# Christopher-Wang/DistriFlow

Hardware: AMD Instinct MI355X
Metric: images/sec (whole node), MNIST CNN sync-SGD at 1/2/4/8 MI355X; async speedup (higher is better)
Workload: dtype bf16; 1 GPU; model=lenet5, global_batch=4096, per_gpu_batch=4096, parallelism=dp1, optimizer=sgd, graph=full, steps_per_graph=64, p2p_reason=single rank, step=train+reduce/update, params=61706

## Files before the change

### csrc/lenet_fused.hip

```cpp
#include "common.h"
#include "diag.h"
#include "kernels.h"
#include "lenet_frag.h"
#include "ll_exchange.h"
#include "optim_device.h"
#include "ps_device.h"

#include <algorithm>
#include <cstdlib>
#include <vector>

namespace dfa {
namespace {

constexpr int IMG = 8;
constexpr int NT = 512;
constexpr int NW = NT / 64;
constexpr int ccdiv(int a, int b) { return (a + b - 1) / b; }
constexpr int XS_ELEMS = IMG * 1024 + 32;
constexpr int OFF_XS = 0;
constexpr int OFF_P1 = OFF_XS + XS_ELEMS * 2;
constexpr int OFF_C1 = OFF_P1 + IMG * 196 * 16;
constexpr int DC2_RS = 104;
constexpr int NM = IMG * DC2_RS;
constexpr int OFF_K = OFF_C1 + IMG * 196 * 4;
constexpr int OFF_PX = OFF_K + 32;
constexpr int OFF_FT = OFF_PX + NM * 2;
constexpr int OFF_W = OFF_FT + 98 * 2 * 16;
constexpr int OFF_KZ = OFF_W + 128;
constexpr int OFF_U = OFF_KZ + 32;
constexpr int OFF_XS1 = OFF_U + 32;
constexpr int LD0 = 424, LD1 = 136, LD2 = 104, LD3 = 40;
constexpr int OFF_H0 = OFF_U;
constexpr int OFF_H1 = OFF_H0 + IMG * LD0 * 2;
constexpr int OFF_H2 = OFF_H1 + IMG * LD1 * 2;
constexpr int OFF_Z3 = OFF_H2 + IMG * LD2 * 2;
constexpr int OFF_Z2 = OFF_Z3 + IMG * LD3 * 2;
constexpr int OFF_Z1 = OFF_Z2 + IMG * LD2 * 2;
constexpr int OFF_ZR = OFF_Z1 + IMG * LD1 * 2;
constexpr int OFF_LG = OFF_ZR + LD0 * 2;
constexpr int OFF_C2 = OFF_LG + IMG * 16 * 4;
constexpr int U_DENSE = OFF_C2 + IMG * 25 * 16 - OFF_U;
constexpr int OFF_DC2 = OFF_U;
constexpr int U_DC2 = NM * 16 * 2;
constexpr int OFF_RED = OFF_XS1 + XS_ELEMS * 2;
constexpr int U_G = 32 + XS_ELEMS * 2 + 4 * 16 * 32 * 4;
__device__ __forceinline__ int dc2_swz(int t) { return t ^ ((t >> 3) & 7); }
constexpr int cmax(int a, int b) { return a > b ? a : b; }
constexpr int NFP1 = (FR_C2 - FR_C1) * 64, NFP2 = (FR_DG - FR_C2) * 64;
constexpr int OFF_FC1 = OFF_XS1;
constexpr int OFF_FC2 = OFF_U + U_DENSE;
constexpr int U_FC2 = U_DENSE + NFP2 * 16;
static_assert(FR_C1 == 0 && FR_C2 - FR_C1 == 15 && FR_DG - FR_C2 == 7, "phase 0 stages fragments 0 .. 21 as one range");
static_assert(OFF_FC1 + NFP1 * 16 <= OFF_XS1 + (XS_ELEMS / 8 - 1) * 16, "build_shift1 overwrites the conv1 fragments");
constexpr int OFF_DB = OFF_U + (cmax(cmax(cmax(U_DENSE, U_DC2), U_G), U_FC2) + 15) / 16 * 16;
constexpr int OFF_ST = OFF_DB + 864;
constexpr int LDS_BYTES = OFF_ST + 128;
static_assert(OFF_U == OFF_C1 + IMG * 196 * 4 + 128 + 98 * 2 * 16 + 800 * 2 + 128 && OFF_U % 16 == 0 && OFF_KZ % 16 == 0 && OFF_H1 % 16 == 0 && OFF_ZR % 16 == 0 && OFF_C2 % 16 == 0 && OFF_RED % 16 == 0 && OFF_DB % 16 == 0 && OFF_ST % 16 == 0 &&
                  OFF_PX % 16 == 0 && OFF_W % 16 == 0 && OFF_FC1 % 16 == 0 && OFF_FC2 % 16 == 0,
              "LDS carve must stay 16-byte aligned");
static_assert(2 * LDS_BYTES <= 160 * 1024, "two workgroups per CU");

typedef __bf16 bf16x4_vs __attribute__((__vector_size__(8)));

#define LN_STAMP(slot)                                                            \
  do {                                                                            \
    if (stamps) {                                                                 \
      __builtin_amdgcn_sched_barrier(0);                                          \
      unsigned long long t_;                                                      \
      asm volatile("s_memtime %0\n\ts_waitcnt lgkmcnt(0)" : "=s"(t_)::"memory"); \
      __builtin_amdgcn_sched_barrier(0);                                          \
      if (threadIdx.x == 0) STMP[(slot)] = t_;                                    \
    }                                                                             \
  } while (0)

template <int CTRL>
__device__ __forceinline__ float dpp_f(float v) {
  return __builtin_bit_cast(float, __builtin_amdgcn_update_dpp(0, __builtin_bit_cast(int, v), CTRL, 0xf, 0xf, false));
}
__device__ __forceinline__ float row16_max(float v) {
  v = fmaxf(v, dpp_f<0xB1>(v));
  v = fmaxf(v, dpp_f<0x4E>(v));
  v = fmaxf(v, dpp_f<0x141>(v));
  return fmaxf(v, dpp_f<0x140>(v));
}
__device__ __forceinline__ float row16_sum(float v) {
  v += dpp_f<0xB1>(v);
  v += dpp_f<0x4E>(v);
  v += dpp_f<0x141>(v);
  return v + dpp_f<0x140>(v);
}

__device__ __forceinline__ bf16x4 tr_read(const bf16* p) {
  auto* lp = (__attribute__((address_space(3))) bf16*)(const_cast<bf16*>(p));
  const bf16x4_vs v =
      __builtin_amdgcn_ds_read_tr16_b64_v4bf16(reinterpret_cast<__attribute__((address_space(3))) bf16x4_vs*>(lp));
  return __builtin_bit_cast(bf16x4, v);
}
__device__ __forceinline__ bf16x8 cat8(bf16x4 a, bf16x4 b) {
  bf16x8 r;
#pragma unroll
  for (int e = 0; e < 4; ++e) {
    r[e] = a[e];
    r[e + 4] = b[e];
  }
  return r;
}
__device__ __forceinline__ bf16x8 ld8(const bf16* p) { return *reinterpret_cast<const bf16x8*>(p); }
__device__ __forceinline__ void st8(bf16* p, const bf16x8& v) { *reinterpret_cast<bf16x8*>(p) = v; }
__device__ __forceinline__ bf16x8 zero8() {
  bf16x8 z;
#pragma unroll
  for (int e = 0; e < 8; ++e) z[e] = (bf16)0.f;
  return z;
}

__device__ __forceinline__ void build_shift1(const bf16* Xs, bf16* Xs1) {
  for (int t = threadIdx.x; t < XS_ELEMS / 8 - 1; t += NT) {
    const uint4 lo = *reinterpret_cast<const uint4*>(Xs + 8 * t);
    const unsigned nx = *reinterpret_cast<const unsigned*>(Xs + 8 * t + 8);
    uint4 o;
    o.x = __builtin_amdgcn_alignbyte(lo.y, lo.x, 2);
    o.y = __builtin_amdgcn_alignbyte(lo.z, lo.y, 2);
    o.z = __builtin_amdgcn_alignbyte(lo.w, lo.z, 2);
    o.w = __builtin_amdgcn_alignbyte(nx, lo.w, 2);
    *reinterpret_cast<uint4*>(Xs1 + 8 * t) = o;
  }
}

__device__ __forceinline__ void pool4(float a00, float a01, float a10, float a11, float& best, unsigned& code) {
  best = a00;
  code = 0;
  if (a01 > best) { best = a01; code = 1; }
  if (a10 > best) { best = a10; code = 2; }
  if (a11 > best) { best = a11; code = 3; }
  if (!(best > 0.f)) { best = 0.f; code = 4; }
}

template <int KS, int NTW>
struct DenseFrags {
  bf16x8 b[NTW][KS];
};
template <int KS, int NTW>
__device__ __forceinline__ void dense_load(DenseFrags<KS, NTW>& f, const bf16x8* __restrict__ W, int ntiles) {
  const int lane = threadIdx.x & 63, w = threadIdx.x >> 6;
#pragma unroll
  for (int tt = 0; tt < NTW; ++tt) {
    const int t = w + NW * tt;
    if (t < ntiles) {
#pragma unroll
      for (int s = 0; s < KS; ++s) f.b[tt][s] = W[(t * KS + s) * 64 + lane];
    }
  }
}

__device__ __forceinline__ void act_store4(bf16* __restrict__ T, int ldt, int n, int c0, int nlive, const float (&v)[4]) {
  if (nlive >= 4) {
    bf16x4 pk;
#pragma unroll
    for (int r = 0; r < 4; ++r) pk[r] = f2bf(v[r]);
    *reinterpret_cast<bf16x4*>(T + lenet_act_pos(n, c0, ldt)) = pk;
  } else {
    for (int r = 0; r < 4; ++r)
      if (r < nlive) T[lenet_act_pos(n, c0 + r, ldt)] = f2bf(v[r]);
  }
}

template <int KS, int NTW>
__device__ __forceinline__ void dense_fwd(const DenseFrags<KS, NTW>& f, const bf16* A, int lda, const bf16* zr,
                                          const float* __restrict__ bias, int N, bool relu, bf16* out, int ldo,
                                          float* out32, bf16* __restrict__ hT, int ldt, int r0, int rows) {
  const int lane = threadIdx.x & 63, w = threadIdx.x >> 6, i = lane & 15, g = lane >> 4;
  const int ntiles = (N + 15) / 16;
  const bf16* arow = (i < IMG ? A + i * lda : zr) + 8 * g;
#pragma unroll
  for (int tt = 0; tt < NTW; ++tt) {
    const int t = w + NW * tt;
    if (t >= ntiles) break;
    const int n = 16 * t + i;
    f32x4 acc = {0.f, 0.f, 0.f, 0.f};
#pragma unroll
    for (int s = 0; s < KS; ++s) acc = mfma16x16x32(ld8(arow + 32 * s), f.b[tt][s], acc);
    if (g >= 2) continue;
    const float bv = (bias != nullptr && n < N) ? bias[n] : 0.f;
    float v[4];
#pragma unroll
    for (int r = 0; r < 4; ++r) {
      v[r] = acc[r] + bv;
      if (relu) v[r] = fmaxf(v[r], 0.f);
      if (n >= N) v[r] = 0.f;
      const int row = 4 * g + r;
      if (out) out[row * ldo + n] = f2bf(v[r]);
      if (out32) out32[row * 16 + (n & 15)] = v[r];
    }
    if (hT != nullptr && n < N) act_store4(hT, ldt, n, r0 + 4 * g, rows - 4 * g, v);
  }
}

template <int KS, int NTW>
__device__ __forceinline__ void dense_bwd(const DenseFrags<KS, NTW>& f, const bf16* dZ, int ldz, const bf16* zr,
                                          int K, const bf16* mask, int ldm, bf16* out, int ldo,
                                          bf16* __restrict__ gT, int ldt, int r0, int rows) {
  const int lane = threadIdx.x & 63, w = threadIdx.x >> 6, i = lane & 15, g = lane >> 4;
  const int ktiles = (K + 15) / 16;
  const bf16* zrow = (i < IMG ? dZ + i * ldz : zr) + 8 * g;
#pragma unroll
  for (int tt = 0; tt < NTW; ++tt) {
    const int t = w + NW * tt;
    if (t >= ktiles) break;
    const int j = 16 * t + i;
    f32x4 acc = {0.f, 0.f, 0.f, 0.f};
#pragma unroll
    for (int s = 0; s < KS; ++s) acc = mfma16x16x32(ld8(zrow + 32 * s), f.b[tt][s], acc);
    if (g >= 2) continue;
    float v[4];
#pragma unroll
    for (int r = 0; r < 4; ++r) {
      const int row = 4 * g + r;
      v[r] = acc[r];
      if (mask != nullptr && !((float)mask[row * ldm + j] > 0.f)) v[r] = 0.f;
      if (j >= K) v[r] = 0.f;
      out[row * ldo + j] = f2bf(v[r]);
    }
    if (gT != nullptr && j < K) act_store4(gT, ldt, j, r0 + 4 * g, rows - 4 * g, v);
  }
}

__device__ __forceinline__ int lenet_img_group(int b, int nb) {
  const int per = nb / 8;
  if (b >= 8 * per) return b;
  return (b & 7) * per + (b >> 3);
}

__device__ __forceinline__ void lenet_ps_owner_decide(const PSArgs& p, unsigned* s_cnt) {
  const int k = threadIdx.x;
  if (k < p.nshards) {
    const unsigned ep = __hip_atomic_load(p.scratch + kPSEpoch, __ATOMIC_RELAXED, __HIP_MEMORY_SCOPE_AGENT) + 1u;
    const unsigned R = (unsigned)p.owner_ring;
    const unsigned pre = __hip_atomic_load(p.pref + k, __ATOMIC_RELAXED, __HIP_MEMORY_SCOPE_SYSTEM);
    unsigned P = 0, n = 0, c = pre, free_ = 0;
    if (__hip_atomic_compare_exchange_strong(p.dlock + k, &free_, (unsigned)p.rank + 1u, __ATOMIC_RELAXED,
                                             __ATOMIC_RELAXED, __HIP_MEMORY_SCOPE_SYSTEM)) {
      P = __hip_atomic_load(p.pref + k, __ATOMIC_RELAXED, __HIP_MEMORY_SCOPE_SYSTEM);
      const unsigned* fl = ps_inbox_flags(p, k);
      while (n < R && n < 255u &&
             __hip_atomic_load(const_cast<unsigned*>(fl) + (P + n) % R, __ATOMIC_RELAXED, __HIP_MEMORY_SCOPE_SYSTEM) ==
                 P + n + 1u)
        ++n;
      if (n == 0) __hip_atomic_store(p.dlock + k, 0u, __ATOMIC_RELAXED, __HIP_MEMORY_SCOPE_SYSTEM);
      c = P + n;
    }
    __hip_atomic_store(ps_owner_drain_words(p) + k, ps_owner_word(ep, n, P), __ATOMIC_RELAXED, __HIP_MEMORY_SCOPE_AGENT);
    s_cnt[k] = c;
  }
  __syncthreads();
  if (threadIdx.x == 0) {
    unsigned cnt = 0xffffffffu;
    for (int j = 0; j < p.nshards; ++j) cnt = s_cnt[j] < cnt ? s_cnt[j] : cnt;
    const unsigned dec = __hip_atomic_load(p.scratch + kPSDecision, __ATOMIC_RELAXED, __HIP_MEMORY_SCOPE_AGENT) & 7u;
    if (dec == kPSAccept && cnt == p.scratch[kPSSeq]) cnt += 1u;
    if (dec == kPSAccept || dec == kPSReject) ps_note_refresh(p, cnt);
  }
}

__device__ __forceinline__ void lenet_ps_admission(const PSArgs& p, bool excl) {
  const long long bid = *p.bid_out;
  const unsigned applied0 = ps_read_applied(p);
  const unsigned ep = __hip_atomic_load(p.scratch + kPSEpoch, __ATOMIC_RELAXED, __HIP_MEMORY_SCOPE_AGENT) + 1u;
  const unsigned dec = ps_admit(p, false);
  const bool owner = p.owner_ring > 0;
  if (!owner && (dec == kPSAccept || dec == kPSReject)) ps_note_refresh(p, applied0 + (dec == kPSAccept ? 1u : 0u));
  __hip_atomic_store(p.scratch + kPSDecision, (ep << 3) | dec, __ATOMIC_RELAXED, __HIP_MEMORY_SCOPE_AGENT);
  if (excl) {
    __hip_atomic_store(p.scratch + kPSEpoch, ep, __ATOMIC_RELAXED, __HIP_MEMORY_SCOPE_AGENT);
    if (dec == kPSAccept) ps_publish_applied(p);
  }
  if (dec == kPSAccept && p.done_epoch != nullptr) complete_microbatch(p, bid);
}

template <bool TRIM>
__global__ void __launch_bounds__(NT, 2 * NT / 256) lenet_train_kernel(LeNetArgs a) {
  if ((int)blockIdx.x >= a.nblk) {
    if (a.ps_admit && threadIdx.x == 0) lenet_ps_admission(a.ps, a.ps_excl != 0);
    return;
  }
  extern __shared__ __attribute__((aligned(16))) char smem[];
  bf16* Xs = reinterpret_cast<bf16*>(smem + OFF_XS);
  bf16* Xs1 = reinterpret_cast<bf16*>(smem + OFF_XS1);
  bf16* P1 = reinterpret_cast<bf16*>(smem + OFF_P1);
  unsigned* C1 = reinterpret_cast<unsigned*>(smem + OFF_C1);
  bf16* KO = reinterpret_cast<bf16*>(smem + OFF_K);
  unsigned char* FT = reinterpret_cast<unsigned char*>(smem + OFF_FT);
  unsigned short* PX = reinterpret_cast<unsigned short*>(smem + OFF_PX);
  float* WS = reinterpret_cast<float*>(smem + OFF_W);
  bf16* H0 = reinterpret_cast<bf16*>(smem + OFF_H0);
  bf16* H1 = reinterpret_cast<bf16*>(smem + OFF_H1);
  bf16* H2 = reinterpret_cast<bf16*>(smem + OFF_H2);
  bf16* Z3 = reinterpret_cast<bf16*>(smem + OFF_Z3);
  bf16* Z2 = reinterpret_cast<bf16*>(smem + OFF_Z2);
  bf16* Z1 = reinterpret_cast<bf16*>(smem + OFF_Z1);
  bf16* ZR = reinterpret_cast<bf16*>(smem + OFF_ZR);
  float* LG = reinterpret_cast<float*>(smem + OFF_LG);
  unsigned char* C2 = reinterpret_cast<unsigned char*>(smem + OFF_C2);
  bf16* DC2 = reinterpret_cast<bf16*>(smem + OFF_DC2);
  float* RED = reinterpret_cast<float*>(smem + OFF_RED);

  const int tid = threadIdx.x, lane = tid & 63, w = __builtin_amdgcn_readfirstlane(tid >> 6), i = lane & 15,
            g = lane >> 4;
  const int r0 = lenet_img_group(blockIdx.x, a.nblk) * (TRIM ? a.ipw : IMG);
  const int rows = min(TRIM ? a.ipw : IMG, a.B - r0);
  const int nA = TRIM ? 2 * ((7 * rows + 1) / 2) : 56;
  const int nB = TRIM ? (13 * rows + 1) / 2 : NM / 16;
  const int nE = TRIM ? ((13 * rows + 3) / 4 + 1) / 2 * 2 : NM / 32;
  const int nF = TRIM ? (49 * rows + 7) / 8 : 49;
  const int nG = TRIM ? 14 * rows : IMG * 14;
  const bf16x8* __restrict__ frag = reinterpret_cast<const bf16x8*>(a.frag);
  float* part = a.conv_part + (long long)blockIdx.x * kLeNetConvStride;
  unsigned long long* const stamps = a.stamps;
  unsigned long long* const STMP = reinterpret_cast<unsigned long long*>(smem + OFF_ST);
  LN_STAMP(0);

  const int ximg = tid / 28, xrow = tid - 28 * (tid / 28);
  const bool xload = tid < IMG * 28 && ximg < rows;
  const bool lload = tid >= 256 && tid < 256 + IMG && tid - 256 < rows;
  long long xsrc = 0, lsrc = 0;
  if (xload) xsrc = a.idx ? a.idx[r0 + ximg] : (long long)(r0 + ximg);
  if (lload) lsrc = a.idx ? a.idx[r0 + tid - 256] : (long long)(r0 + tid - 256);
  uint4 tabv = {0u, 0u, 0u, 0u};
  if (tid < 98 * 2) tabv = reinterpret_cast<const uint4*>(a.ftab)[tid];
  else if (tid >= 264 && tid < 264 + NM / 8) tabv = reinterpret_cast<const uint4*>(a.pxtab)[tid - 264];
  static_assert(98 * 2 <= 256 && 264 + NM / 8 <= 448 && 448 + 22 <= NT, "phase 0 staging thread ranges");
  float biasv = 0.f, dbv = 0.f;
  if (tid >= 448 && tid < 448 + 22) biasv = *(tid < 454 ? a.b1 + (tid - 448) : a.b2 + (tid - 454));
  if (tid < 214) dbv = *(tid < 120 ? a.d1b + tid : (tid < 204 ? a.d2b + (tid - 120) : a.d3b + (tid - 204)));
  constexpr int NFK = ccdiv(NFP1 + NFP2, NT);
  bf16x8 fv[NFK];
#pragma unroll
  for (int k = 0; k < NFK; ++k) fv[k] = frag[FR_C1 * 64 + min(tid + NT * k, NFP1 + NFP2 - 1)];
  const int lbl = a.labels[lsrc < 0 ? 0 : (lsrc >= a.nrows ? a.nrows - 1 : lsrc)];
  unsigned xv[14];
  {
    const long long src = xsrc < 0 ? 0 : (xsrc >= a.nrows ? a.nrows - 1 : xsrc);
    const int xr = xload ? xrow : 0;
    if (a.x_u8 != nullptr) {
      const unsigned* p = reinterpret_cast<const unsigned*>(a.x_u8 + src * 784 + xr * 28);
#pragma unroll
      for (int k = 0; k < 7; ++k) xv[k] = p[k];
    } else {
      const uint2* p = reinterpret_cast<const uint2*>(a.x_bf + src * 784 + xr * 28);
#pragma unroll
      for (int k = 0; k < 7; ++k) {
        const uint2 v = p[k];
        xv[2 * k] = v.x;
        xv[2 * k + 1] = v.y;
      }
    }
  }
  const bf16x8 z8 = zero8();
  bf16x8 one6 = z8;
  one6[6] = (bf16)1.f;
  for (int e = tid; e < (OFF_K - OFF_XS) / 16; e += NT)
    st8(Xs + 8 * e, (e >= OFF_P1 / 16 && e < OFF_C1 / 16) ? one6 : z8);
  static_assert(OFF_FC2 + NFP2 * 16 == OFF_DB, "the conv2 fragment image ends the union");
  if (tid < (OFF_FC1 - OFF_U) / 16) st8(reinterpret_cast<bf16*>(smem + OFF_U) + 8 * tid, z8);
  for (int e = (OFF_FC1 - OFF_U) / 16 + NFP1 + tid; e < (OFF_FC2 - OFF_U) / 16; e += NT)
    st8(reinterpret_cast<bf16*>(smem + OFF_U) + 8 * e, z8);
#pragma unroll
  for (int k = 0; k < NFK; ++k) {
    const int p = tid + NT * k;
    if (p < NFP1) st8(reinterpret_cast<bf16*>(smem + OFF_FC1) + 8 * p, fv[k]);
    else if (p < NFP1 + NFP2) st8(reinterpret_cast<bf16*>(smem + OFF_FC2) + 8 * (p - NFP1), fv[k]);
  }
  if (tid < 2) {
    bf16x8 o;
#pragma unroll
    for (int e = 0; e < 8; ++e) o[e] = (bf16)1.f;
    st8(KO + 8 * tid, o);
  } else if (tid < 4) {
    st8(reinterpret_cast<bf16*>(smem + OFF_KZ) + 8 * (tid - 2), z8);
  }
  if (tid < 98 * 2) reinterpret_cast<uint4*>(FT)[tid] = tabv;
  else if (tid >= 264 && tid < 264 + NM / 8) reinterpret_cast<uint4*>(PX)[tid - 264] = tabv;
  if (tid >= 448 && tid < 448 + 22) WS[tid - 448] = biasv;
  float* DB = reinterpret_cast<float*>(smem + OFF_DB);
  if (tid < 214) DB[tid] = dbv;
  int* LBL = reinterpret_cast<int*>(WS + 24);
  if (tid >= 256 && tid < 256 + IMG) LBL[tid - 256] = lbl;
  __syncthreads();
  bf16x8 bc[15];
#pragma unroll
  for (int f = 0; f < 15; ++f) bc[f] = ld8(reinterpret_cast<const bf16*>(smem + OFF_FC1) + 8 * (f * 64 + lane));
  if (xload) {
    unsigned* dst = reinterpret_cast<unsigned*>(Xs + ximg * 1024 + (xrow + 2) * 32 + 2);
    if (a.x_u8 != nullptr) {
#pragma unroll
      for (int k = 0; k < 7; ++k)
#pragma unroll
        for (int h = 0; h < 2; ++h) {
          const float f0 = (float)((xv[k] >> (16 * h)) & 255u) * a.scale;
          const float f1 = (float)((xv[k] >> (16 * h + 8)) & 255u) * a.scale;
          const unsigned lo = __builtin_bit_cast(unsigned short, f2bf(f0));
          const unsigned hi = __builtin_bit_cast(unsigned short, f2bf(f1));
          dst[2 * k + h] = lo | (hi << 16);
        }
    } else {
#pragma unroll
      for (int k = 0; k < 14; ++k) dst[k] = xv[k];
    }
  }
  __syncthreads();
  build_shift1(Xs, Xs1);
  __syncthreads();
  LN_STAMP(1);

  {
    const float b1c[3] = {WS[(i >> 3)], WS[2 + (i >> 3)], WS[4 + (i >> 3)]};
#pragma unroll 2
    for (int u = w; u < nA; u += NT / 64) {
      const int mt = u >> 1, x0 = (u & 1) * 16;
      const int m = 16 * mt + i;
      const int img = m / 56, rem = m - 56 * (m / 56);
      const bf16* abase = ((rem & 1) ? Xs1 : Xs) + img * 1024 + (rem >> 1) * 32 + x0 + 8 * g;
      f32x4 acc[3];
#pragma unroll
      for (int T = 0; T < 3; ++T) acc[T] = {0.f, 0.f, 0.f, 0.f};
#pragma unroll
      for (int ky = 0; ky < 5; ++ky) {
        const bf16x8 av = ld8(abase + ky * 32);
#pragma unroll
        for (int T = 0; T < 3; ++T) acc[T] = mfma16x16x32(av, bc[ky * 3 + T], acc[T]);
      }
      const int m0 = 16 * mt + 4 * g;
      const int imgo = m0 / 56, py = (m0 - 56 * (m0 / 56)) >> 2;
      const int px = (x0 >> 1) + (i & 7);
      unsigned cw = 0;
#pragma unroll
      for (int T = 0; T < 3; ++T) {
        float best;
        unsigned code;
        pool4(acc[T][0] + b1c[T], acc[T][1] + b1c[T], acc[T][2] + b1c[T], acc[T][3] + b1c[T], best, code);
        const int c = 2 * T + (i >> 3);
        if (px < 14) P1[((imgo * 14 + py) * 14 + px) * 8 + c] = f2bf(best);
        cw |= code << (3 * c);
      }
      cw |= __shfl_xor(cw, 8, 64);
      if (i < 8 && px < 14) C1[(imgo * 14 + py) * 14 + px] = cw;
    }
  }
  __syncthreads();
  LN_STAMP(2);

  bf16x8 bw[7];
#pragma unroll
  for (int s = 0; s < 7; ++s) bw[s] = ld8(reinterpret_cast<const bf16*>(smem + OFF_FC2) + 8 * (s * 64 + lane));
  DenseFrags<13, ccdiv(8, NW)> f1;
  dense_load(f1, frag + FR_D1W * 64, 8);
  {
    int toff[7];
#pragma unroll
    for (int s = 0; s < 7; ++s) {
      const int tap = 4 * s + g;
      toff[s] = tap < 25 ? ((tap / 5) * 14 + (tap - 5 * (tap / 5))) * 8 : 0;
    }
    const float b2 = WS[6 + i];
#pragma unroll 2
    for (int mt = w; mt < nB; mt += NT / 64) {
      const bf16* abase = P1 + (int)PX[16 * mt + i] * 8;
      f32x4 acc = {0.f, 0.f, 0.f, 0.f};
#pragma unroll
      for (int s = 0; s < 7; ++s) acc = mfma16x16x32(ld8(abase + toff[s]), bw[s], acc);
      const int m0 = 16 * mt + 4 * g;
      const int img0 = m0 / DC2_RS, win0 = (m0 - DC2_RS * img0) >> 2;
      float best;
      unsigned code;
      pool4(acc[0] + b2, acc[1] + b2, acc[2] + b2, acc[3] + b2, best, code);
      if (win0 < 25) {
        H0[img0 * LD0 + win0 * 16 + i] = f2bf(best);
        C2[(img0 * 25 + win0) * 16 + i] = (unsigned char)code;
      }
    }
  }
  __syncthreads();
  LN_STAMP(3);

  for (int k = tid; k < 400; k += NT) {
    if (rows == IMG) {
      bf16x8 v;
#pragma unroll
      for (int r = 0; r < IMG; ++r) v[r] = H0[r * LD0 + k];
      st8(a.h0T + lenet_act_pos(k, r0, a.ldt), v);
    } else {
      for (int r = 0; r < rows; ++r) a.h0T[lenet_act_pos(k, r0 + r, a.ldt)] = H0[r * LD0 + k];
    }
  }
  DenseFrags<4, ccdiv(6, NW)> f2;
  DenseFrags<3, 1> f3;
  dense_load(f2, frag + FR_D2W * 64, 6);
  dense_load(f3, frag + FR_D3W * 64, 1);
  dense_fwd(f1, H0, LD0, ZR, DB, 120, true, H1, LD1, nullptr, a.h1T, a.ldt, r0, rows);
  __syncthreads();
  DenseFrags<1, ccdiv(6, NW)> g3;
  DenseFrags<3, ccdiv(8, NW)> g2;
  dense_load(g3, frag + FR_D3WT * 64, 6);
  dense_load(g2, frag + FR_D2WT * 64, 8);
  dense_fwd(f2, H1, LD1, ZR, DB + 120, 84, true, H2, LD2, nullptr, a.h2T, a.ldt, r0, rows);
  __syncthreads();
  dense_fwd(f3, H2, LD2, ZR, DB + 204, 10, false, nullptr, 0, LG, nullptr, a.ldt, r0, rows);
  __syncthreads();
  LN_STAMP(4);
  if (tid < IMG * 16) {
    const int r = tid >> 4, c = tid & 15;
    const bool live = r < rows;
    const int y = min(max(LBL[r], 0), 9);
    const float z = c < 10 ? LG[r * 16 + c] : -INFINITY;
    if (a.logits && live && c < 10) a.logits[(long long)(r0 + r) * 10 + c] = z;
    const float mx = row16_max(z);
    const unsigned long long hit = __ballot(z == mx);
    const int am = __builtin_ctzll((hit >> (16 * (r & 3))) | 0x10000ull);
    const float e = c < 10 ? __expf(z - mx) : 0.f;
    const float ssum = row16_sum(e);
    if (live && c < 10) {
      const float gv = (e * (1.f / ssum) - (c == y ? 1.f : 0.f)) * a.grad_scale;
      Z3[r * LD3 + c] = f2bf(gv);
      a.dz3T[lenet_act_pos(c, r0 + r, a.ldt)] = f2bf(gv);
    }
    if (c == y) LG[r * 16 + 14] = live ? -(z - mx - __logf(ssum)) : 0.f;
    if (c == 15) LG[r * 16 + 15] = (live && am == y) ? 1.f : 0.f;
  }
  __syncthreads();
  if (tid == 0) {
    float ls = 0.f, cs = 0.f;
#pragma unroll
    for (int r = 0; r < IMG; ++r) {
      ls += LG[r * 16 + 14];
      cs += LG[r * 16 + 15];
    }
    a.loss_part[2 * blockIdx.x] = ls;
    a.loss_part[2 * blockIdx.x + 1] = cs;
  }
  DenseFrags<4, ccdiv(25, NW)> g1;
  dense_load(g1, frag + FR_D1WT * 64, 25);
  __syncthreads();
  LN_STAMP(5);
  dense_bwd(g3, Z3, LD3, ZR, 84, H2, LD2, Z2, LD2, a.dz2T, a.ldt, r0, rows);
  __syncthreads();
  dense_bwd(g2, Z2, LD2, ZR, 120, H1, LD1, Z1, LD1, a.dz1T, a.ldt, r0, rows);
  __syncthreads();
  dense_bwd(g1, Z1, LD1, ZR, 400, H0, LD0, H0, LD0, nullptr, 0, r0, rows);
  __syncthreads();
  LN_STAMP(6);

  {
    bf16x8 dp[2];
    unsigned long long cd[2];
#pragma unroll
    for (int k = 0; k < 2; ++k) {
      const int it = tid + k * NT;
      if (it < IMG * 50) {
        const int img = it / 50, rem = it - 50 * (it / 50), win = rem >> 1, nh = rem & 1;
        dp[k] = ld8(H0 + img * LD0 + win * 16 + 8 * nh);
        cd[k] = *reinterpret_cast<const unsigned long long*>(C2 + (img * 25 + win) * 16 + 8 * nh);
      }
    }
    __syncthreads();
#pragma unroll
    for (int k = 0; k < 2; ++k) {
      const int it = tid + k * NT;
      if (it < IMG * 50) {
        const int img = it / 50, rem = it - 50 * (it / 50), win = rem >> 1, nh = rem & 1;
#pragma unroll
        for (int d = 0; d < 4; ++d) {
          bf16x8 o;
#pragma unroll
          for (int e = 0; e < 8; ++e) o[e] = ((cd[k] >> (8 * e)) & 255u) == (unsigned)d ? dp[k][e] : (bf16)0.f;
          st8(DC2 + ((img * DC2_RS + dc2_swz(win * 4 + d)) * 16 + 8 * nh), o);
        }
      }
    }
  }
  if (tid < IMG * 8) {
    const int img = tid >> 3, rr = (tid >> 1) & 3, nh = tid & 1;
    st8(DC2 + ((img * DC2_RS + dc2_swz(100 + rr)) * 16 + 8 * nh), zero8());
  }
  __syncthreads();
  LN_STAMP(7);

  bf16x8 bd[15];
#pragma unroll
  for (int s = 0; s < 15; ++s) bd[s] = frag[(FR_DG + s) * 64 + lane];
  {
    const int q = (lane & 15) >> 2, p = lane & 3;
    constexpr int KT = ccdiv(13, NW);
    int toff[KT];
#pragma unroll
    for (int k = 0; k < KT; ++k) {
      const int tap = 2 * (w + NW * k) + (p >> 1);
      toff[k] = tap < 25 ? ((tap / 5) * 14 + (tap - 5 * (tap / 5))) * 8 + 4 * (p & 1) : 4 * (p & 1);
    }
    const int ntile = (13 - w + NW - 1) / NW;
    f32x4 acc[KT];
#pragma unroll
    for (int k = 0; k < KT; ++k) acc[k] = {0.f, 0.f, 0.f, 0.f};
    auto ldAv = [&](int s) -> bf16x8 {
      const int mA = 32 * s + 8 * g + q;
      const int b = 4 * s + g, sx = (b - 13 * ((b * 79) >> 10)) & 7;
      return cat8(tr_read(DC2 + (mA ^ sx) * 16 + 4 * p), tr_read(DC2 + ((mA + 4) ^ sx) * 16 + 4 * p));
    };
    auto step = [&](const bf16x8& av, unsigned px0, unsigned px1) {
      const bf16* pb0 = P1 + 8 * px0;
      const bf16* pb1 = P1 + 8 * px1;
      bf16x4 t0[KT], t1[KT];
#pragma unroll
      for (int k = 0; k < KT; ++k) {
        t0[k] = tr_read(pb0 + toff[k]);
        t1[k] = tr_read(pb1 + toff[k]);
      }
#pragma unroll
      for (int k = 0; k < KT; ++k) acc[k] = mfma16x16x32(av, cat8(t0[k], t1[k]), acc[k]);
    };
    static_assert(NM / 32 % 2 == 0, "phase E pairs its steps");
    const unsigned short* pxl = PX + 8 * g + q;
    bf16x8 ava = ldAv(0);
    unsigned pxa0 = pxl[0], pxa1 = pxl[4];
#pragma unroll 1
    for (int s = 0; s < nE; s += 2) {
      const bf16x8 avb = ldAv(s + 1);
      const unsigned pxb0 = pxl[32 * (s + 1)], pxb1 = pxl[32 * (s + 1) + 4];
      __builtin_amdgcn_sched_barrier(0);
      step(ava, pxa0, pxa1);
      __builtin_amdgcn_sched_barrier(0);
      const int sn = s + 2 < nE ? s + 2 : s;
      ava = ldAv(sn);
      pxa0 = pxl[32 * sn];
      pxa1 = pxl[32 * sn + 4];
      __builtin_amdgcn_sched_barrier(0);
      step(avb, pxb0, pxb1);
      __builtin_amdgcn_sched_barrier(0);
    }
#pragma unroll
    for (int k = 0; k < KT; ++k) {
      if (k < ntile) {
        const int T = w + NW * k;
        const int tap = 2 * T + (i >> 3), c = i & 7;
#pragma unroll
        for (int r = 0; r < 4; ++r) {
          const int n = 4 * g + r;
          if (tap < 25 && c < 6) part[(long long)(kLeNetPW2 + n * 150 + tap * 6 + c)] = acc[k][r];
          else if (tap == 0 && c == 6) part[(long long)(kLeNetPB2 + n)] = acc[k][r];
        }
      }
    }
  }
  __syncthreads();
  LN_STAMP(8);

  {
    const int bcol = i >> 3, c = i & 7;
#pragma unroll 2
    for (int mt = w; mt < nF; mt += NT / 64) {
      const int m = 16 * mt + i;
      const int img = m / 98, rem = m - 98 * (m / 98);
      const uint4 tv = *reinterpret_cast<const uint4*>(FT + (rem * 2 + (g >> 1)) * 16);
      const unsigned tw[4] = {tv.x, tv.y, tv.z, tv.w};
      const unsigned dbase = (unsigned)OFF_DC2 + 16u * (unsigned)(g & 1) + 32u * (unsigned)(img * DC2_RS);
      auto ldA = [&](int st) -> bf16x8 {
        const unsigned t = (tw[st >> 2] >> (8 * (st & 3))) & 255u;
        return *reinterpret_cast<const bf16x8*>(smem + dbase + 32u * t);
      };
      f32x4 acc = {0.f, 0.f, 0.f, 0.f};
      bf16x8 a0 = ldA(0), a1 = ldA(1), a2 = ldA(2);
#pragma unroll
      for (int s = 0; s < 15; ++s) {
        acc = mfma16x16x32(a0, bd[s], acc);
        a0 = a1;
        a1 = a2;
        if (s + 3 < 15) a2 = ldA(s + 3);
      }
      if (c < 6) {
#pragma unroll
        for (int r = 0; r < 4; ++r) {
          const int mm = 16 * mt + 4 * g + r;
          P1[(2 * mm + bcol) * 8 + c] = f2bf(acc[r]);
        }
      }
    }
  }
  __syncthreads();
  build_shift1(Xs, Xs1);
  __syncthreads();
  LN_STAMP(9);

  {
    f32x4 acc[2] = {{0.f, 0.f, 0.f, 0.f}, {0.f, 0.f, 0.f, 0.f}};
    const int gdy = i >= 6 && i < 12 ? 1 : 0;
    const int ca = i < 6 ? i : (i < 12 ? i - 6 : 5);
    constexpr int kXs1 = (OFF_XS1 - OFF_XS) / 2;
    unsigned boff[2], bconst[2];
    bool breal[2];
#pragma unroll
    for (int T = 0; T < 2; ++T) {
      const int e = 16 * T + i;
      const int ep = e < 30 ? e : 0;
      const int ky = ep / 5, kx = ep - 5 * (ep / 5);
      boff[T] = 2u * (unsigned)(((kx & 1) ? kXs1 : 0) + ky * 32 + 8 * g + 2 * (kx >> 1));
      breal[T] = e < 30;
      bconst[T] = e == 30 ? (unsigned)OFF_K : (unsigned)OFF_KZ;
    }
    unsigned cmask[4];
#pragma unroll
    for (int wd = 0; wd < 4; ++wd) cmask[wd] = (4 * g + wd < 14 && i < 12) ? 0u : 8u;
#pragma unroll 2
    for (int rp = w; rp < nG; rp += NT / 64) {
      const int img = rp / 14, py = rp - 14 * (rp / 14);
      const int p0 = (img * 14 + py) * 14 + 4 * g;
      const uint2 cA = *reinterpret_cast<const uint2*>(C1 + p0);
      const uint2 cB = *reinterpret_cast<const uint2*>(C1 + p0 + 2);
      const unsigned cw[4] = {cA.x, cA.y, cB.x, cB.y};
      unsigned aw[4];
#pragma unroll
      for (int wd = 0; wd < 4; ++wd) {
        const unsigned sel = (((cw[wd] >> (3 * ca)) & 7u) | cmask[wd]) - 2u * (unsigned)gdy;
        const unsigned pv = *reinterpret_cast<const unsigned short*>(P1 + (p0 + wd) * 8 + ca);
        aw[wd] = sel < 2u ? pv << (sel << 4) : 0u;
      }
      const bf16x8 av = __builtin_bit_cast(bf16x8, uint4{aw[0], aw[1], aw[2], aw[3]});
      const unsigned rowb = (unsigned)OFF_XS + 2u * (unsigned)(img * 1024 + 2 * py * 32);
#pragma unroll
      for (int T = 0; T < 2; ++T) {
        const unsigned* bp = reinterpret_cast<const unsigned*>(smem + (breal[T] ? rowb + boff[T] : bconst[T]));
        const bf16x8 bv = __builtin_bit_cast(bf16x8, uint4{bp[0], bp[1], bp[2], bp[3]});
        acc[T] = mfma16x16x32(av, bv, acc[T]);
      }
    }
    if (w >= 4) {
#pragma unroll
      for (int T = 0; T < 2; ++T)
#pragma unroll
        for (int r = 0; r < 4; ++r) RED[((w & 3) * 16 + 4 * g + r) * 32 + 16 * T + i] = acc[T][r];
    }
    __syncthreads();
    if (w < 4) {
#pragma unroll
      for (int T = 0; T < 2; ++T)
#pragma unroll
        for (int r = 0; r < 4; ++r) {
          float* q = RED + (w * 16 + 4 * g + r) * 32 + 16 * T + i;
          *q = (NW > 4 ? *q : 0.f) + acc[T][r];
        }
    }
    __syncthreads();
    auto S = [&](int row, int col) {
      return RED[(0 * 16 + row) * 32 + col] + RED[(1 * 16 + row) * 32 + col] + RED[(2 * 16 + row) * 32 + col] +
             RED[(3 * 16 + row) * 32 + col];
    };
    for (int e = tid; e < 6 * 26; e += NT) {
      const int c = e / 26, t = e - 26 * (e / 26);
      if (t < 25) part[(long long)(kLeNetPW1 + c * 25 + t)] = S(c, t) + S(6 + c, t + 5);
      else part[(long long)(kLeNetPB1 + c)] = S(c, 30) + S(6 + c, 30);
    }
  }
  LN_STAMP(10);
  if (stamps && tid < 11) stamps[blockIdx.x * 16 + tid] = STMP[tid];
}

constexpr int PT = 1024;
constexpr int kPrepBlocks = 1 + ccdiv(kLeNetDenseFragLanes, PT);
__global__ void __launch_bounds__(PT) lenet_prep_kernel(const float* __restrict__ w1g, const float* __restrict__ w2g,
                                                        const float* __restrict__ d1g, const float* __restrict__ d2g,
                                                        const float* __restrict__ d3g, bf16x8* __restrict__ frag) {
  if (blockIdx.x > 0) {
    const int dl = (blockIdx.x - 1) * PT + threadIdx.x;
    if (dl < kLeNetDenseFragLanes)
      frag[kLeNetFragLanes + dl] =
          lenet_dense_frag_lane(dl, [&](int l, int j) { return (l == 0 ? d1g : (l == 1 ? d2g : d3g))[j]; });
    return;
  }
  __shared__ float w[kLeNetConvW];
  for (int e = threadIdx.x; e < 150; e += PT) w[e] = w1g[e];
  for (int e = threadIdx.x; e < 2400; e += PT) w[150 + e] = w2g[e];
  __syncthreads();
  lenet_build_frags(w, frag, threadIdx.x, PT);
}

constexpr int RT = 256;
constexpr int kDU = 32;
constexpr int kChunks = 8;
constexpr int kConvPer = 256;
constexpr int kSlotVals = 1024;
constexpr int kPerThread = kSlotVals / RT;
constexpr int kMaxOwned = 16;
constexpr unsigned long long kSuccTimeoutTicks = 100000000ull;
static_assert(kSlotVals <= kLLSlot, "LL slot too small");

struct Owned {
  int di, i;
};

struct RedTables : LeNetRedTab {
  float hyper[5];
};

__device__ __forceinline__ void stage_tables(const LeNetRedArgs& a, RedTables* t) {
  constexpr int kWords = (int)(sizeof(LeNetRedTab) / 4);
  static_assert(sizeof(LeNetRedTab) % 4 == 0 && kWords <= RT, "table image");
  typedef const __attribute__((address_space(4))) char kchar;
  typedef const __attribute__((address_space(4))) int kint;
  kint* src = (kint*)((kchar*)__builtin_amdgcn_kernarg_segment_ptr() + offsetof(LeNetRedArgs, tab));
  if ((int)threadIdx.x < kWords) reinterpret_cast<int*>(static_cast<LeNetRedTab*>(t))[threadIdx.x] = src[threadIdx.x];
  if (a.sgd_on && threadIdx.x >= 64 && threadIdx.x < 69) t->hyper[threadIdx.x - 64] = a.sgd.hyper[threadIdx.x - 64];
}

__device__ __forceinline__ int dense_unit(const RedTables& t, int u, int& tn, int& tk) {
  int l = 0;
  if (u >= t.L[0].tiles) {
    u -= t.L[0].tiles;
    l = 1;
    if (u >= t.L[1].tiles) {
      u -= t.L[1].tiles;
      l = 2;
    }
  }
  const int nt = (t.L[l].N + kDU - 1) / kDU;
  tk = u / nt;
  tn = u - nt * tk;
  return l;
}

__device__ __forceinline__ int slot_dense(const LeNetRedArgs& a, int slot) {
  return slot >= a.nconv_slots ? slot - a.nconv_slots : -1;
}
__device__ __forceinline__ int slot_conv(const LeNetRedArgs& a, int slot) { return slot; }

__device__ __forceinline__ Owned owned_elem(const LeNetRedArgs& a, const RedTables& t, int slot, int pos) {
  const int du = slot_dense(a, slot);
  if (du >= 0) {
    int tn, tk;
    const int l = dense_unit(t, du, tn, tk);
    const int N = t.L[l].N, K = t.L[l].K;
    const int on = kDU * tn + (pos >> 5), ok = kDU * tk + (pos & 31);
    if (on >= N || ok > K) return {-1, 0};
    return ok < K ? Owned{4 + 2 * l, on * K + ok} : Owned{5 + 2 * l, on};
  }
  const int p = slot_conv(a, slot) * kConvPer + pos;
  if (pos >= kConvPer || p >= kLeNetConvParams) return {-1, 0};
  if (p < kLeNetPB1) return {0, p};
  if (p < kLeNetPW2) return {1, p - kLeNetPB1};
  if (p < kLeNetPB2) return {2, p - kLeNetPW2};
  return {3, p - kLeNetPB2};
}

__device__ __forceinline__ int conv_wj(Owned o) { return o.di == 0 ? o.i : o.di == 2 ? 150 + o.i : -1; }

__device__ __forceinline__ void dense_job(const LeNetRedArgs& a, const RedTables& t, int u, int c, float* red,
                                          float (&out)[kPerThread], int nch = kChunks) {
  const int lane = threadIdx.x & 63, wid = __builtin_amdgcn_readfirstlane(threadIdx.x >> 6);
  int tn, tk;
  const int l = dense_unit(t, u, tn, tk);
  const LeNetDense& L = t.L[l];
  const int cw = nch == 1 ? a.kcols : a.chunk_cols;
  const int col0 = c * cw, col1 = min(a.kcols, col0 + cw);
  const bf16* arow[2];
  const bf16* brow[2];
  bool a_ok[2], b_ok[2], b_one[2];
  const int kb = a.ldt >> 5;
#pragma unroll
  for (int i = 0; i < 2; ++i) {
    const int n = kDU * tn + 16 * i + (lane & 15), k = kDU * tk + 16 * i + (lane & 15);
    const int ta = min(2 * tn + i, (L.N + 15) / 16 - 1), tb = min(2 * tk + i, (L.K + 15) / 16 - 1);
    arow[i] = L.dzT + (((long long)ta * kb + (col0 >> 5)) * 64 + lane) * 8;
    brow[i] = L.hT + (((long long)tb * kb + (col0 >> 5)) * 64 + lane) * 8;
    a_ok[i] = n < L.N;
    b_ok[i] = k < L.K;
    b_one[i] = k == L.K;
  }
  bf16x8 ones, zeros = zero8();
#pragma unroll
  for (int e = 0; e < 8; ++e) ones[e] = (bf16)1.f;
  const int steps = col1 > col0 ? (col1 - col0) / 32 : 0;
  const int per = (steps + 3) / 4;
  const int s0 = wid * per, s1 = min(steps, s0 + per);
  f32x4 acc[2][2];
#pragma unroll
  for (int i = 0; i < 2; ++i)
#pragma unroll
    for (int j = 0; j < 2; ++j) acc[i][j] = f32x4{0.f, 0.f, 0.f, 0.f};
  for (int s = s0; s < s1; s += 4) {
    bf16x8 av[2][4], bv[2][4];
#pragma unroll
    for (int q = 0; q < 4; ++q) {
      const int ss = min(s + q, s1 - 1);
#pragma unroll
      for (int i = 0; i < 2; ++i) {
        av[i][q] = ld8(arow[i] + 512 * ss);
        bv[i][q] = ld8(brow[i] + 512 * ss);
      }
    }
#pragma unroll
    for (int q = 0; q < 4; ++q) {
      const bool live = s + q < s1;
#pragma unroll
      for (int i = 0; i < 2; ++i)
#pragma unroll
        for (int j = 0; j < 2; ++j)
          acc[i][j] = mfma16x16x32((a_ok[i] && live) ? av[i][q] : zeros,
                                   b_ok[j] ? bv[j][q] : (b_one[j] ? ones : zeros), acc[i][j]);
    }
  }
#pragma unroll
  for (int i = 0; i < 2; ++i)
#pragma unroll
    for (int j = 0; j < 2; ++j)
#pragma unroll
      for (int r = 0; r < 4; ++r)
        red[wid * kSlotVals + (16 * i + 4 * (lane >> 4) + r) * kDU + 16 * j + (lane & 15)] = acc[i][j][r];
  __syncthreads();
#pragma unroll
  for (int e = 0; e < kPerThread; ++e) {
    const int pos = threadIdx.x + RT * e;
    out[e] = ((red[pos] + red[kSlotVals + pos]) + red[2 * kSlotVals + pos]) + red[3 * kSlotVals + pos];
  }
}

__device__ __forceinline__ void conv_job(const LeNetRedArgs& a, int s, int c, float* red, float (&out)[kPerThread],
                                         int nch = kChunks) {
  const int lane = threadIdx.x & 63, wid = __builtin_amdgcn_readfirstlane(threadIdx.x >> 6);
  const int p0 = s * kConvPer + 4 * lane;
  const int pl = min(p0, kLeNetConvStride - 4);
  const int nrows = a.nblk > c ? (a.nblk - 1 - c) / nch + 1 : 0;
  f32x4 acc = {0.f, 0.f, 0.f, 0.f};
  for (int i0 = wid; i0 < nrows; i0 += 4 * 16) {
    f32x4 v[16];
#pragma unroll
    for (int k = 0; k < 16; ++k) {
      const int i = min(i0 + 4 * k, nrows - 1);
      v[k] = *reinterpret_cast<const f32x4*>(a.conv_part + (long long)(c + nch * i) * kLeNetConvStride + pl);
    }
#pragma unroll
    for (int k = 0; k < 16; ++k)
      if (i0 + 4 * k < nrows) acc += v[k];
  }
  *reinterpret_cast<f32x4*>(red + wid * kSlotVals + 4 * lane) = acc;
  __syncthreads();
  const int pos = threadIdx.x;
  out[0] = ((red[pos] + red[kSlotVals + pos]) + red[2 * kSlotVals + pos]) + red[3 * kSlotVals + pos];
#pragma unroll
  for (int e = 1; e < kPerThread; ++e) out[e] = 0.f;
}

template <bool DENSE>
__device__ __forceinline__ void red_emit(const LeNetRedArgs& a, const RedTables& t, Owned o, float w) {
  const ParamDesc& d = t.d[o.di];
// ... 997 lines not shown
```

Measured before the change: 81.26 million images/s.

## Split conv2 weight-gradient reduction across two K-halves of waves

The conv2 weight-gradient phase previously gave each of 8 waves up to 2 column tiles and swept the full reduction dimension. Now the waves form 2 halves by 4 column groups. Each half reduces over half of the K steps, with 3 or 4 tiles per wave, and the two halves' accumulators are combined through LDS in the P1 buffer before the partial sums are written. The aim is to balance per-wave MFMA work and cut the serial K loop length. The cost is an extra LDS round trip, two block barriers, and higher accumulator register pressure. The step count no longer rounds up to an even number, and dead rows' gradient entries in Z3 are now zero-filled.

```diff
diff --git a/csrc/lenet_fused.hip b/csrc/lenet_fused.hip
--- a/csrc/lenet_fused.hip
+++ b/csrc/lenet_fused.hip
@@ -8,6 +8,7 @@
 
 #include <algorithm>
 #include <cstdlib>
+#include <type_traits>
 #include <vector>
 
 namespace dfa {
@@ -311,7 +312,7 @@
   const int rows = min(TRIM ? a.ipw : IMG, a.B - r0);
   const int nA = TRIM ? 2 * ((7 * rows + 1) / 2) : 56;
   const int nB = TRIM ? (13 * rows + 1) / 2 : NM / 16;
-  const int nE = TRIM ? ((13 * rows + 3) / 4 + 1) / 2 * 2 : NM / 32;
+  const int nE = TRIM ? (13 * rows + 3) / 4 : NM / 32;
   const int nF = TRIM ? (49 * rows + 7) / 8 : 49;
   const int nG = TRIM ? 14 * rows : IMG * 14;
   const bf16x8* __restrict__ frag = reinterpret_cast<const bf16x8*>(a.frag);
@@ -519,10 +520,10 @@
     const int am = __builtin_ctzll((hit >> (16 * (r & 3))) | 0x10000ull);
     const float e = c < 10 ? __expf(z - mx) : 0.f;
     const float ssum = row16_sum(e);
-    if (live && c < 10) {
-      const float gv = (e * (1.f / ssum) - (c == y ? 1.f : 0.f)) * a.grad_scale;
+    if (c < 10) {
+      const float gv = live ? (e * (1.f / ssum) - (c == y ? 1.f : 0.f)) * a.grad_scale : 0.f;
       Z3[r * LD3 + c] = f2bf(gv);
-      a.dz3T[lenet_act_pos(c, r0 + r, a.ldt)] = f2bf(gv);
+      if (live) a.dz3T[lenet_act_pos(c, r0 + r, a.ldt)] = f2bf(gv);
     }
     if (c == y) LG[r * 16 + 14] = live ? -(z - mx - __logf(ssum)) : 0.f;
     if (c == 15) LG[r * 16 + 15] = (live && am == y) ? 1.f : 0.f;
@@ -590,63 +591,86 @@
   for (int s = 0; s < 15; ++s) bd[s] = frag[(FR_DG + s) * 64 + lane];
   {
     const int q = (lane & 15) >> 2, p = lane & 3;
-    constexpr int KT = ccdiv(13, NW);
-    int toff[KT];
-#pragma unroll
-    for (int k = 0; k < KT; ++k) {
-      const int tap = 2 * (w + NW * k) + (p >> 1);
-      toff[k] = tap < 25 ? ((tap / 5) * 14 + (tap - 5 * (tap / 5))) * 8 + 4 * (p & 1) : 4 * (p & 1);
-    }
-    const int ntile = (13 - w + NW - 1) / NW;
-    f32x4 acc[KT];
-#pragma unroll
-    for (int k = 0; k < KT; ++k) acc[k] = {0.f, 0.f, 0.f, 0.f};
+    const int h = w >> 2, cg = w & 3;
+    constexpr int KTM = ccdiv(13, NW / 2);
+    static_assert(NW == 8 && KTM == 4, "phase E: 2 K-halves x 4 column groups of 4, 3, 3, 3 tiles");
+    const int nlo = (nE + 1) >> 1;
+    const int sb = h ? nlo : 0, se = h ? nE : nlo;
+    const int ntile = cg == 0 ? KTM : KTM - 1;
+    f32x4 acc[KTM];
+#pragma unroll
+    for (int k = 0; k < KTM; ++k) acc[k] = {0.f, 0.f, 0.f, 0.f};
     auto ldAv = [&](int s) -> bf16x8 {
       const int mA = 32 * s + 8 * g + q;
       const int b = 4 * s + g, sx = (b - 13 * ((b * 79) >> 10)) & 7;
       return cat8(tr_read(DC2 + (mA ^ sx) * 16 + 4 * p), tr_read(DC2 + ((mA + 4) ^ sx) * 16 + 4 * p));
     };
-    auto step = [&](const bf16x8& av, unsigned px0, unsigned px1) {
-      const bf16* pb0 = P1 + 8 * px0;
-      const bf16* pb1 = P1 + 8 * px1;
-      bf16x4 t0[KT], t1[KT];
+    const unsigned short* pxl = PX + 8 * g + q;
+    auto run = [&](auto ktc) {
+      constexpr int KT = decltype(ktc)::value;
+      int toff[KT];
 #pragma unroll
       for (int k = 0; k < KT; ++k) {
-        t0[k] = tr_read(pb0 + toff[k]);
-        t1[k] = tr_read(pb1 + toff[k]);
-      }
-#pragma unroll
-      for (int k = 0; k < KT; ++k) acc[k] = mfma16x16x32(av, cat8(t0[k], t1[k]), acc[k]);
+        const int tap = 2 * (cg + NW / 2 * k) + (p >> 1);
+        toff[k] = tap < 25 ? ((tap / 5) * 14 + (tap - 5 * (tap / 5))) * 8 + 4 * (p & 1) : 4 * (p & 1);
+      }
+      auto step = [&](const bf16x8& av, unsigned px0, unsigned px1) {
+        const bf16* pb0 = P1 + 8 * px0;
+        const bf16* pb1 = P1 + 8 * px1;
+        bf16x4 t0[KT], t1[KT];
+#pragma unroll
+        for (int k = 0; k < KT; ++k) {
+          t0[k] = tr_read(pb0 + toff[k]);
+          t1[k] = tr_read(pb1 + toff[k]);
+        }
+#pragma unroll
+        for (int k = 0; k < KT; ++k) acc[k] = mfma16x16x32(av, cat8(t0[k], t1[k]), acc[k]);
+      };
+      bf16x8 ava = ldAv(sb);
+      unsigned pxa0 = pxl[32 * sb], pxa1 = pxl[32 * sb + 4];
+      int s = sb;
+#pragma unroll 1
+      for (; s + 1 < se; s += 2) {
+        const bf16x8 avb = ldAv(s + 1);
+        const unsigned pxb0 = pxl[32 * (s + 1)], pxb1 = pxl[32 * (s + 1) + 4];
+        __builtin_amdgcn_sched_barrier(0);
+        step(ava, pxa0, pxa1);
+        __builtin_amdgcn_sched_barrier(0);
+        const int sn = s + 2 < se ? s + 2 : s;
+        ava = ldAv(sn);
+        pxa0 = pxl[32 * sn];
+        pxa1 = pxl[32 * sn + 4];
+        __builtin_amdgcn_sched_barrier(0);
+        step(avb, pxb0, pxb1);
+        __builtin_amdgcn_sched_barrier(0);
+      }
+      if (s < se) step(ava, pxa0, pxa1);
     };
-    static_assert(NM / 32 % 2 == 0, "phase E pairs its steps");
-    const unsigned short* pxl = PX + 8 * g + q;
-    bf16x8 ava = ldAv(0);
-    unsigned pxa0 = pxl[0], pxa1 = pxl[4];
-#pragma unroll 1
-    for (int s = 0; s < nE; s += 2) {
-      const bf16x8 avb = ldAv(s + 1);
-      const unsigned pxb0 = pxl[32 * (s + 1)], pxb1 = pxl[32 * (s + 1) + 4];
-      __builtin_amdgcn_sched_barrier(0);
-      step(ava, pxa0, pxa1);
-      __builtin_amdgcn_sched_barrier(0);
-      const int sn = s + 2 < nE ? s + 2 : s;
-      ava = ldAv(sn);
-      pxa0 = pxl[32 * sn];
-      pxa1 = pxl[32 * sn + 4];
-      __builtin_amdgcn_sched_barrier(0);
-      step(avb, pxb0, pxb1);
-      __builtin_amdgcn_sched_barrier(0);
-    }
-#pragma unroll
-    for (int k = 0; k < KT; ++k) {
-      if (k < ntile) {
-        const int T = w + NW * k;
-        const int tap = 2 * T + (i >> 3), c = i & 7;
-#pragma unroll
-        for (int r = 0; r < 4; ++r) {
-          const int n = 4 * g + r;
-          if (tap < 25 && c < 6) part[(long long)(kLeNetPW2 + n * 150 + tap * 6 + c)] = acc[k][r];
-          else if (tap == 0 && c == 6) part[(long long)(kLeNetPB2 + n)] = acc[k][r];
+    if (cg == 0) run(std::integral_constant<int, KTM>{});
+    else run(std::integral_constant<int, KTM - 1>{});
+    static_assert(13 * 64 * 16 <= IMG * 196 * 16, "the upper half's 13 accumulator tiles fit in P1");
+    f32x4* ES = reinterpret_cast<f32x4*>(smem + OFF_P1);
+    __syncthreads();
+    if (h) {
+#pragma unroll
+      for (int k = 0; k < KTM; ++k)
+        if (k < ntile) ES[(cg + NW / 2 * k) * 64 + lane] = acc[k];
+    }
+    __syncthreads();
+    if (!h) {
+#pragma unroll
+      for (int k = 0; k < KTM; ++k) {
+        if (k < ntile) {
+          const int T = cg + NW / 2 * k;
+          const f32x4 up = ES[T * 64 + lane];
+          const int tap = 2 * T + (i >> 3), c = i & 7;
+#pragma unroll
+          for (int r = 0; r < 4; ++r) {
+            const int n = 4 * g + r;
+            const float v = acc[k][r] + up[r];
+            if (tap < 25 && c < 6) part[(long long)(kLeNetPW2 + n * 150 + tap * 6 + c)] = v;
+            else if (tap == 0 && c == 6) part[(long long)(kLeNetPB2 + n)] = v;
+          }
         }
       }
     }
```

New measurement: 83.47 million images/s (median of 6 runs). +2.7%, better.
